# bioinfologics/w2rap-contigger

Hardware: AMD Instinct MI355X
Metric: step2_k60_canonical_kmers_per_s (higher is better)
Workload: dtype u64

## Files before the change

### w2rap_contigger_amd/csrc/step2_count.hip

```cpp
#include <algorithm>
#include <chrono>
#include <cstdlib>
#include <cstring>
#include <type_traits>
#include "ctx.h"

namespace w2 {

constexpr unsigned QSLOTS = 256;
template <bool MASK>
__global__ void __launch_bounds__(256) k_good_len(uint64_t n, const uint8_t* __restrict__ quals, const uint32_t* __restrict__ qmask,
                                                   const uint64_t* __restrict__ qoff, const uint32_t* __restrict__ len,
                                                   uint32_t min_qual, uint16_t* __restrict__ good,
                                                   unsigned long long* __restrict__ total_kmers,
                                                   uint32_t* __restrict__ max_len) {
    constexpr unsigned CH = 4096;
    __shared__ __attribute__((aligned(16))) uint16_t gbits[CH + 16];
    __shared__ unsigned long long s_sum[4];
    __shared__ uint32_t s_max[4];
    const uint64_t r0 = (uint64_t)blockIdx.x * blockDim.x;
    const uint64_t r = r0 + threadIdx.x;
    const uint64_t rend = r0 + blockDim.x < n ? r0 + blockDim.x : n;
    const uint64_t base0 = qoff[r0], endo = qoff[rend];
    const unsigned shift = MASK ? (unsigned)(base0 & 31) : (unsigned)((reinterpret_cast<uintptr_t>(quals) + base0) & 15);
// ... 949 lines not shown
                        const unsigned long long pos = gb + run + (unsigned)__builtin_popcountll(sm[j] & ((1ull << lane) - 1));
                        if (pos < solid_cap) { shi[pos] = keys[2 * i]; slo[pos] = keys[2 * i + 1]; scc[pos] = vals[j] & 0xFFFFu; }
                        keys[2 * i] = EMPTY; keys[2 * i + 1] = EMPTY;
                    }
                    run += (unsigned)__builtin_popcountll(sm[j]);
                }
            }
            tick(5);
            if (sp == 0) break;
            __syncthreads();
        }
    }
    __syncthreads();
    if (tid == 0) { misc[K3_BASELO] = (uint32_t)pend_base; misc[K3_BASEHI] = (uint32_t)(pend_base >> 32); }
    __syncthreads();
    {
        const uint32_t nprev = misc[K3_NPREV];
        const unsigned long long pk = (unsigned long long)misc[K3_BASELO] | ((unsigned long long)misc[K3_BASEHI] << 32);
        const unsigned long long gb = pk & SMASK;
        for (unsigned i = tid; i < nprev; i += THREADS)
            if (gb + i < solid_cap) { shi[gb + i] = sthi[i]; slo[gb + i] = stlo[i]; scc[gb + i] = stcc[i]; }
        if (tid == 0 && nprev && chunk_start && (pk >> 40) < chunk_cap) { chunk_start[pk >> 40] = gb; chunk_cnt[pk >> 40] = nprev; }
    }
    for (unsigned i = tid; i < 101; i += THREADS) if (lhist[i]) atomicAdd(&ghist[i], (unsigned long long)lhist[i]);
    for (int o = 32; o > 0; o >>= 1) my_distinct += __shfl_down(my_distinct, o);
    if (lane == 0 && my_distinct) atomicAdd(&counters[1], my_distinct);
    if (PROF && tid == 0) { for (int i = 0; i < 6; ++i) atomicAdd(&counters[106 + i], pt[i]); atomicAdd(&counters[112], ptmax);
                            for (int i = 0; i < 5; ++i) atomicAdd(&counters[113 + i], wt[i]); }
    if (PROF && lane == 0) atomicAdd(&counters[124 + wv], wcount);
}

#ifdef W2RAP_FP_TS9
constexpr unsigned FP_TS = REC_DWORDS | 1u;
#else
constexpr unsigned FP_TS = REC_DWORDS;
#endif
__device__ inline unsigned fp_tile_index(unsigned d) { return FP_TS == REC_DWORDS ? d : d + d / REC_DWORDS; }
template <unsigned THREADS, unsigned TILE_, unsigned SC_>
struct FpCfg {
    static constexpr unsigned CAP = 4096, LOG_CAP = 12, NW = THREADS / 64;
    static constexpr unsigned TILE = TILE_;
    static constexpr unsigned ROUNDS = (TILE + THREADS - 1) / THREADS;
    static constexpr unsigned MAXK = 16384, MAXWIN = MAXK / 64;
    static constexpr unsigned PFREC = TILE < 512 ? TILE : 512;
    static constexpr unsigned NPF = (PFREC * REC_DWORDS + THREADS - 1) / THREADS;
    static constexpr unsigned SC = SC_;
    static constexpr unsigned QCAP = 128;
    static constexpr unsigned MAXSEG = 16;
    static constexpr unsigned LIMIT = CAP - THREADS - 8 < 3072 ? CAP - THREADS - 8 : 3072;
    static constexpr unsigned PER = CAP / THREADS;
    static constexpr unsigned OCAP = CAP;
    static constexpr unsigned LDS = 3 * MAXSEG * 8 +
                                    (2 * CAP + TILE * FP_TS + 8 + MAXK / 32 + 2 + MAXWIN + 2 + 2 * SC + NW * QCAP + 3 * (MAXSEG + 1) + 32 + 4 + 104 + 16 + 40 + (OCAP + 1) / 2) * 4;
    static_assert(TILE < 1023 && ROUNDS * NW <= 16 && (1u << LOG_CAP) == CAP, "FpCfg");
};
enum { FP_FILL = 0, FP_OVF, FP_CNT, FP_BASELO, FP_BASEHI, FP_WIN, FP_DEPTH };
#ifndef W2RAP_FP_TICKETS
#define W2RAP_FP_TICKETS 4
#endif
constexpr uint32_t FP_TICKETS = W2RAP_FP_TICKETS;
static_assert((FP_TICKETS & (FP_TICKETS - 1)) == 0, "FP_TICKETS");

struct FpInst {
    uint32_t s[4];
    uint32_t e0, e3;
};
__device__ inline FpInst fp_fetch(const uint32_t* tile, unsigned rec, unsigned idx) {
    const uint32_t* wp = tile + rec * FP_TS;
    const unsigned q0 = (idx + REC_HB / 2) >> 4, sh = ((idx + REC_HB / 2) & 15u) * 2u;
    const uint32_t d0 = wp[q0], d1 = wp[1 + q0], d2 = wp[2 + q0], d3 = wp[3 + q0], d4 = wp[4 + q0];
    FpInst x;
    const uint32_t e0 = __funnelshift_r(d0, d1, sh), e1 = __funnelshift_r(d1, d2, sh), e2 = __funnelshift_r(d2, d3, sh), e3 = __funnelshift_r(d3, d4, sh);
    x.s[0] = __funnelshift_r(e0, e1, 2); x.s[1] = (e1 >> 2) & 0x0FFFFFFFu;
    x.s[2] = __funnelshift_r(e1, e2, 30); x.s[3] = __funnelshift_r(e2, e3, 30) & 0x0FFFFFFFu;
    x.e0 = e0; x.e3 = e3;
    return x;
}
struct FpKey { uint64_t hi, lo; bool rc; uint32_t f[4]; };
__device__ inline FpKey fp_key(const FpInst& x) {
    auto rev2_32 = [](uint32_t v) { v = __brev(v); return ((v & 0x55555555u) << 1) | ((v >> 1) & 0x55555555u); };
    const uint32_t a0 = rev2_32(x.s[0]), b0 = rev2_32(x.s[1]), a1 = rev2_32(x.s[2]), b1 = rev2_32(x.s[3]);
    FpKey k;
    k.f[0] = a0 >> 4; k.f[1] = __funnelshift_r(b0, a0, 4); k.f[2] = a1 >> 4; k.f[3] = __funnelshift_r(b1, a1, 4);
    const uint64_t khi_f = ((uint64_t)k.f[0] << 32) | k.f[1], klo_f = ((uint64_t)k.f[2] << 32) | k.f[3];
    const uint64_t khi_r = ((uint64_t)(~x.s[3] & 0x0FFFFFFFu) << 32) | (uint32_t)~x.s[2], klo_r = ((uint64_t)(~x.s[1] & 0x0FFFFFFFu) << 32) | (uint32_t)~x.s[0];
    k.rc = khi_r != khi_f ? khi_r < khi_f : klo_r < klo_f;
    k.hi = k.rc ? khi_r : khi_f; k.lo = k.rc ? klo_r : klo_f;
    return k;
}
__device__ inline uint32_t fp_hash(const FpKey& k) {
    const uint32_t fa = (uint32_t)k.hi ^ (uint32_t)(k.lo >> 32), fb = (uint32_t)(k.hi >> 32) ^ (uint32_t)k.lo;
    return (fa + ((fb << 16) | (fb >> 16))) * 0x9E3779B1u;
}
__device__ inline bool fp_same(const uint32_t* tile, unsigned ref, const FpInst& x, const FpKey& k) {
    const FpInst r = fp_fetch(tile, ref >> 6, ref & 63u);
    const uint32_t same = (r.s[0] ^ x.s[0]) | (r.s[1] ^ x.s[1]) | (r.s[2] ^ x.s[2]) | (r.s[3] ^ x.s[3]);
    const uint32_t opp = ((r.s[3] ^ k.f[0]) | 0xF0000000u) & (r.s[2] ^ k.f[1]) & ((r.s[1] ^ k.f[2]) | 0xF0000000u) & (r.s[0] ^ k.f[3]);
    return same == 0u || opp == 0xFFFFFFFFu;
}

template <unsigned THREADS, unsigned MINW, unsigned TILE_, unsigned SC_>
__global__ void __launch_bounds__(THREADS, MINW) k_count_fp(uint32_t nb, uint32_t b_lo, uint32_t b_hi, uint32_t nseg, const uint64_t* __restrict__ roff,
                                                            const uint32_t* __restrict__ recs, uint32_t min_freq, uint32_t* __restrict__ queue,
                                                            uint64_t* __restrict__ shi, uint64_t* __restrict__ slo, uint32_t* __restrict__ scc, uint64_t solid_cap,
                                                            unsigned long long* __restrict__ counters, unsigned long long* __restrict__ ghist,
                                                            uint64_t* __restrict__ chunk_start, uint32_t* __restrict__ chunk_cnt, uint32_t chunk_cap,
                                                            uint32_t* __restrict__ defer , uint32_t defer_cap,
                                                            uint32_t fill_limit , uint32_t solid_limit ,
                                                            uint8_t* __restrict__ sctx, uint8_t* __restrict__ unres, uint32_t* __restrict__ nbr ) {
    constexpr unsigned long long SMASK = (1ull << 40) - 1;
    using C = FpCfg<THREADS, TILE_, SC_>;
    constexpr unsigned CAP = C::CAP, NW = C::NW, TILE = C::TILE, ROUNDS = C::ROUNDS, NPF = C::NPF, SC = C::SC, MAXSEG = C::MAXSEG, PER = C::PER, QCAP = C::QCAP,
                       MAXK = C::MAXK, MAXWIN = C::MAXWIN;
    constexpr uint32_t EMPTY = 0xFFFFFFFFu;
    extern __shared__ __attribute__((aligned(16))) unsigned char smem[];
    uint64_t* segbase = reinterpret_cast<uint64_t*>(smem);
    uint32_t* tab = reinterpret_cast<uint32_t*>(segbase + 3 * MAXSEG);
    uint32_t* cc = tab + CAP;
    uint32_t* tile = cc + CAP;
    uint32_t* bv32 = tile + TILE * FP_TS + 8;
    uint32_t* Bw = bv32 + MAXK / 32 + 2;
    uint32_t* stcc = Bw + MAXWIN + 2;
    uint32_t* stref = stcc + SC;
    uint32_t* qref = stref + SC + (threadIdx.x >> 6) * QCAP;
    uint32_t* segdpre = stref + SC + NW * QCAP;
    uint32_t* wtot = segdpre + 3 * (MAXSEG + 1);
    uint32_t* bq = wtot + 32;
    uint32_t* lhist = bq + 4;
    uint32_t* misc = lhist + 104;
    uint32_t* stk = misc + 16;
    uint16_t* olist = reinterpret_cast<uint16_t*>(stk + 40);
    const unsigned tid = threadIdx.x, lane = tid & 63, wv = tid >> 6;

    auto seg_load = [&](uint32_t bb, uint64_t& r0, uint32_t& cnt) {
        r0 = 0; cnt = 0;
        if (tid < nseg && bb < b_hi) {
            const uint64_t a = roff[(uint64_t)tid * nb + bb], e = roff[(uint64_t)tid * nb + bb + 1];
            r0 = a; cnt = e - a < (1ull << 20) ? (uint32_t)(e - a) : (1u << 20);
        }
    };
    auto seg_store = [&](unsigned q, uint64_t r0, uint32_t cnt) {
        uint32_t incl = cnt;
#pragma unroll
        for (int o = 1; o < 64; o <<= 1) { uint32_t v = __shfl_up(incl, o); if ((int)lane >= o) incl += v; }
        const uint32_t tot = (uint32_t)__builtin_amdgcn_readlane((int)incl, 63);
        const uint32_t ex = incl - cnt;
        if (lane < nseg) { segdpre[q * (MAXSEG + 1) + lane] = ex * REC_DWORDS; segbase[q * MAXSEG + lane] = (r0 - ex) * REC_DWORDS; }
        if (lane == 0) segdpre[q * (MAXSEG + 1) + nseg] = tot * REC_DWORDS;
    };
    auto stream_dword = [&](unsigned q, const uint32_t* dp, const uint32_t (&bnd)[7], uint32_t d) -> uint32_t {
        unsigned s = 0;
        if (nseg <= 8) {
#pragma unroll
            for (unsigned i = 0; i < 7; ++i) s += d >= bnd[i] ? 1u : 0u;
        } else while (d >= dp[s + 1]) ++s;
        return recs[segbase[q * MAXSEG + s] + d];
    };
    auto tile_load = [&](unsigned q, uint32_t (&v)[NPF]) {
        const uint32_t* dp = segdpre + q * (MAXSEG + 1);
        const uint32_t dall = dp[nseg];
        const uint32_t dend = dall < C::PFREC * REC_DWORDS ? dall : C::PFREC * REC_DWORDS;
        uint32_t bnd[7];
#pragma unroll
        for (unsigned i = 0; i < 7; ++i) bnd[i] = (i + 1 < nseg && nseg <= 8) ? dp[i + 1] : 0xFFFFFFFFu;
#pragma unroll
        for (unsigned j = 0; j < NPF; ++j) {
            const uint32_t d = j * THREADS + tid;
            v[j] = d < dend ? stream_dword(q, dp, bnd, d) : 0u;
        }
    };
    auto tile_store = [&](const uint32_t (&v)[NPF]) {
#pragma unroll
        for (unsigned j = 0; j < NPF; ++j) { const unsigned i = j * THREADS + tid; if (i < C::PFREC * REC_DWORDS) tile[fp_tile_index(i)] = v[j]; }
    };
    auto tile_rest = [&](unsigned q) {
        if (TILE <= C::PFREC) return;
        const uint32_t* dp = segdpre + q * (MAXSEG + 1);
        const uint32_t dall = dp[nseg];
        const uint32_t dend = dall < TILE * REC_DWORDS ? dall : TILE * REC_DWORDS;
        uint32_t bnd[7];
#pragma unroll
        for (unsigned i = 0; i < 7; ++i) bnd[i] = (i + 1 < nseg && nseg <= 8) ? dp[i + 1] : 0xFFFFFFFFu;
        for (uint32_t d = C::PFREC * REC_DWORDS + tid; d < dend; d += THREADS) tile[fp_tile_index(d)] = stream_dword(q, dp, bnd, d);
    };
    auto ctx_of = [&](const FpInst& x, bool rc, uint32_t hdr, unsigned idx) -> unsigned {
        const unsigned rnk_ = (hdr & 63u) + 1u;
        const bool hasp = (idx > 0) | ((hdr & 64u) != 0), hass = (idx + 1 < rnk_) | ((hdr & 128u) != 0);
        const unsigned shl_p = (x.e0 & 3u) ^ (rc ? 3u : 4u), shl_s = ((x.e3 >> 26) & 3u) ^ (rc ? 7u : 0u);
        return (hasp ? 1u << shl_p : 0u) | (hass ? 1u << shl_s : 0u);
    };

    for (unsigned i = tid; i < CAP; i += THREADS) { tab[i] = EMPTY; cc[i] = 0; }
    for (unsigned i = tid; i < MAXK / 32 + 2; i += THREADS) bv32[i] = 0;
    for (unsigned i = tid; i < TILE * FP_TS + 8; i += THREADS) tile[i] = 0;
    for (unsigned i = tid; i < 104; i += THREADS) lhist[i] = 0;
    if (tid < 16) misc[tid] = 0;
    if (tid == 0) {
        const uint32_t t0 = atomicAdd(queue, 3u), nbk = b_hi - b_lo;
        bq[0] = t0 < nbk ? b_lo + t0 : NONE32; bq[1] = t0 + 1 < nbk ? b_lo + t0 + 1 : NONE32; bq[2] = t0 + 2 < nbk ? b_lo + t0 + 2 : NONE32; bq[3] = NONE32;
    }
    __syncthreads();
    if (wv == 0) {
        uint64_t r0; uint32_t cnt;
        seg_load(bq[0], r0, cnt); seg_store(0, r0, cnt);
        seg_load(bq[1], r0, cnt); seg_store(1, r0, cnt);
    }
    __syncthreads();
    uint32_t pf[NPF];
    tile_load(0, pf);
    unsigned long long my_distinct = 0;
    unsigned qn = 0;
    uint32_t tick4 = 0;

    auto drain = [&](unsigned cnt) -> unsigned {
        wave_lds_fence();
        const bool live = lane < cnt;
        const unsigned ref = live ? qref[qn - cnt + lane] : 0u;
        const unsigned rec = ref >> 6, idx = ref & 63u;
        const FpInst x = fp_fetch(tile, rec, idx);
        const FpKey k = fp_key(x);
        const unsigned ctx = ctx_of(x, k.rc, tile[rec * FP_TS], idx);
        const uint32_t h1 = fp_hash(k), tag = (h1 >> 5) & 0xFFFFu;
        unsigned s = (h1 >> (33 - C::LOG_CAP)) << 1;
        bool isnew = false;
        if (live) {
            bool ok = false;
            int budget = (int)CAP;
            for (;;) {
                uint32_t a = ld32(&tab[s]);
                if (a == EMPTY) {
                    a = atomicCAS(&tab[s], EMPTY, (tag << 16) | ref);
                    if (a == EMPTY) { isnew = true; ok = true; break; }
                }
                if ((a >> 16) == tag && fp_same(tile, a & 0xFFFFu, x, k)) { ok = true; break; }
                s = (s + 1) & (CAP - 1);
                if (--budget <= 0) break;
            }
            if (ok) { atomicAdd(&cc[s], 1u); atomicOr(&cc[s], ctx << 24); }
            else st32(&misc[FP_OVF], 1u);
        }
        qn -= cnt;
        wave_lds_fence();
        return (unsigned)__builtin_popcountll(__ballot(isnew));
    };

    for (uint32_t it = 0;; ++it) {
        const uint32_t b = (uint32_t)__builtin_amdgcn_readfirstlane((int)ld32(&bq[it & 3]));
        if (b >= b_hi) break;
        const unsigned q = it % 3;
        const uint32_t nrec = (uint32_t)__builtin_amdgcn_readfirstlane((int)segdpre[q * (MAXSEG + 1) + nseg]) / REC_DWORDS;
        bool skip = nrec > TILE;
        tile_store(pf);
        if (!skip) tile_rest(q);
        uint32_t la_b = 0;
        if (tid == 0) {
            if ((it & (FP_TICKETS - 1u)) == 0) tick4 = atomicAdd(queue, FP_TICKETS);
            const uint32_t t = tick4 + (it & (FP_TICKETS - 1u));
            la_b = t < b_hi - b_lo ? b_lo + t : NONE32;
        }
        uint64_t la_r0 = 0; uint32_t la_cnt = 0;
        if (wv == 0) seg_load(ld32(&bq[(it + 2) & 3]), la_r0, la_cnt);
        tile_load((it + 1) % 3, pf);
        __syncthreads();
        unsigned nkr[ROUNDS], inclr[ROUNDS];
#pragma unroll
        for (unsigned r = 0; r < ROUNDS; ++r) {
            const unsigned rec = r * THREADS + tid;
            nkr[r] = (!skip && rec < nrec) ? (tile[rec * FP_TS] & 63u) + 1u : 0u;
            inclr[r] = wave_scan64(nkr[r]);
            if (lane == 63) wtot[r * NW + wv] = inclr[r];
        }
        if (tid == 0) { misc[FP_WIN] = 2 * NW; stk[0] = 0; stk[1] = 1; misc[FP_DEPTH] = 1; }
        __syncthreads();
        const unsigned wsum = lane < ROUNDS * NW ? wtot[lane] : 0u, wsc = row_scan16(wsum);
        const int wvu = __builtin_amdgcn_readfirstlane((int)wv);
        const unsigned total = (unsigned)__builtin_amdgcn_readlane((int)wsc, ROUNDS * NW - 1);
        skip |= total > MAXK;
#pragma unroll
        for (unsigned r = 0; r < ROUNDS; ++r) {
            const unsigned base = (unsigned)__builtin_amdgcn_readlane((int)wsc, r * NW + wvu) - (unsigned)__builtin_amdgcn_readlane((int)wsum, r * NW + wvu);
            if (nkr[r] && !skip) {
                const unsigned e = base + inclr[r] - nkr[r], rec = r * THREADS + tid;
                atomicOr(&bv32[e >> 5], 1u << (e & 31));
                const unsigned w1 = (e + 63) >> 6;
                if (64 * w1 < e + nkr[r]) Bw[w1] = (rec << 16) | e;
            }
        }
        __syncthreads();
        const unsigned nwin = skip ? 0u : (total + 63) / 64;
        bool first_pass = true;
        for (;;) {
        const unsigned sp = (unsigned)__builtin_amdgcn_readfirstlane((int)ld32(&misc[FP_DEPTH])) - 1u;
        const uint32_t cls = (uint32_t)__builtin_amdgcn_readfirstlane((int)stk[2 * sp]), P = (uint32_t)__builtin_amdgcn_readfirstlane((int)stk[2 * sp + 1]);
        {
            uint32_t fill_seen = (uint32_t)__builtin_amdgcn_readfirstlane((int)ld32(&misc[FP_FILL])),
                     ovf_seen = (uint32_t)__builtin_amdgcn_readfirstlane((int)ld32(&misc[FP_OVF]));
            const unsigned wv_s = (unsigned)wvu;
            uint32_t nM0 = 0, nM1 = 0, nB = 0;
            { const unsigned w0 = wv_s < nwin ? wv_s : 0u; nM0 = bv32[2 * w0]; nM1 = bv32[2 * w0 + 1]; nB = Bw[w0]; }
            const uint64_t lane_le = ~0ull >> (63 - lane);
            const uint32_t lane_lt_lo = lane < 32 ? (1u << lane) - 1u : 0xFFFFFFFFu, lane_lt_hi = lane < 32 ? 0u : (1u << (lane - 32)) - 1u;
            unsigned wnext = wv_s + NW;
            for (unsigned w = wv_s; w < nwin;) {
                if (ovf_seen) break;
                if (fill_seen >= fill_limit) { if (lane == 0) st32(&misc[FP_OVF], 1u); break; }
                const uint32_t fill_ld = ld32(&misc[FP_FILL]), ovf_ld = ld32(&misc[FP_OVF]);
                uint32_t wdraw = 0;
                if (lane == 0) wdraw = atomicAdd(&misc[FP_WIN], 1u);
                const uint32_t M0 = nM0, M1 = nM1, Bv = nB;
                { const unsigned wn = wnext < nwin ? wnext : w; nM0 = bv32[2 * wn]; nM1 = bv32[2 * wn + 1]; nB = Bw[wn]; }
                const unsigned g = w * 64 + lane;
                const bool active = g < total;
                const uint32_t mle0 = M0 & (uint32_t)lane_le, mle1 = M1 & (uint32_t)(lane_le >> 32);
                const unsigned c = (unsigned)__builtin_popcount(mle0 & ~1u) + (unsigned)__builtin_popcount(mle1);
                const unsigned top = mle1 ? 63u - (unsigned)__builtin_clz(mle1) : 31u - (unsigned)__builtin_clz(mle0 | 1u);
                const unsigned idx = active ? lane - (c ? top : (Bv & 0xFFFFu) - w * 64) : 0u;
                const unsigned rec = active ? (Bv >> 16) + c : 0u;
                const uint32_t hdr = tile[rec * FP_TS];
                const FpInst x = fp_fetch(tile, rec, idx);
                const FpKey k = fp_key(x);
                const unsigned ctx = ctx_of(x, k.rc, hdr, idx);
                const uint32_t h1 = fp_hash(k), tag = (h1 >> 5) & 0xFFFFu;
                const unsigned s0 = (h1 >> (33 - C::LOG_CAP)) << 1;
                const unsigned myref = (rec << 6) | idx;
                const uint64_t ab = ld64(reinterpret_cast<const uint64_t*>(tab + s0));
                const uint32_t a0 = (uint32_t)ab, a1 = (uint32_t)(ab >> 32);
                const bool m0 = ((a0 >> 16) == tag) & (a0 != EMPTY), m1 = ((a1 >> 16) == tag) & (a1 != EMPTY);
                const bool second = !m0 & (m1 | ((a0 != EMPTY) & (a1 == EMPTY)));
                const uint32_t a = second ? a1 : a0;
                const unsigned s = s0 + (second ? 1u : 0u);
                const bool mine = active & (((h1 >> 2) & (P - 1)) == cls);
                const bool tagm = mine & (m0 | m1);
                const bool hit = tagm & fp_same(tile, tagm ? (a & 0xFFFFu) : myref, x, k);
                const bool want = mine & !tagm & (a == EMPTY);
                const uint32_t old = atomicCAS(&tab[s], EMPTY, want ? ((tag << 16) | myref) : EMPTY);
                const bool won = want & (old == EMPTY);
                const bool done = hit | won;
                atomicAdd(&cc[s], done ? 1u : 0u);
                atomicOr(&cc[s], done ? ctx << 24 : 0u);
                const bool parked = mine & !done;
                unsigned nnew = (unsigned)__builtin_popcountll(__ballot(won));
                {
                    const unsigned long long pm = __ballot(parked);
                    const unsigned below = (unsigned)__builtin_popcount((uint32_t)pm & lane_lt_lo) + (unsigned)__builtin_popcount((uint32_t)(pm >> 32) & lane_lt_hi);
                    const unsigned npark = (unsigned)__builtin_popcountll(pm);
                    qref[qn + (parked ? below : npark + lane - below)] = myref;
                    qn += npark;
                    if (qn >= 64) nnew += drain(64);
                }
                if (nnew && lane == 0) atomicAdd(&misc[FP_FILL], nnew);
                fill_seen = (uint32_t)__builtin_amdgcn_readfirstlane((int)fill_ld); ovf_seen = (uint32_t)__builtin_amdgcn_readfirstlane((int)ovf_ld);
                w = wnext; wnext = (uint32_t)__builtin_amdgcn_readfirstlane((int)wdraw);
            }
            unsigned nnew = 0;
            while (qn) nnew += drain(qn < 64 ? qn : 64);
            if (nnew && lane == 0) atomicAdd(&misc[FP_FILL], nnew);
        }
        if (first_pass) {
            if (wv == 0) seg_store((it + 2) % 3, la_r0, la_cnt);
            if (tid == 0) st32(&bq[(it + 3) & 3], la_b);
            first_pass = false;
        }
        if (tid == 0) {
            misc[FP_CNT] = 0;
            if (skip) misc[FP_OVF] = 1;
        }
        __syncthreads();
        bool deferred = ld32(&misc[FP_OVF]) != 0;
        static_assert(PER % 4 == 0, "PER");
        uint32_t occm = 0, nsol = 0;
        if (!deferred) {
            const u32x4* c4 = reinterpret_cast<const u32x4*>(cc + tid * PER);
#pragma unroll
            for (unsigned j4 = 0; j4 < PER / 4; ++j4) {
                const u32x4 v4 = c4[j4];
#pragma unroll
                for (unsigned j = 0; j < 4; ++j) {
                    const uint32_t cnt = v4[j] & 0xFFFFFFu;
                    occm |= (cnt != 0 ? 1u : 0u) << (4 * j4 + j);
                    nsol += (cnt != 0 && cnt >= min_freq) ? 1u : 0u;
                }
            }
        }
        const unsigned nocc = (unsigned)__builtin_popcount(occm);
        const unsigned i_occ = wave_scan64(nocc), i_sol = wave_scan64(nsol);
        if (lane == 63) { wtot[wv] = i_occ; wtot[16 + wv] = i_sol; }
        __syncthreads();
        const unsigned ws_o = lane < NW ? wtot[lane] : 0u, wc_o = row_scan16(ws_o), ws_s = lane < NW ? wtot[16 + lane] : 0u, wc_s = row_scan16(ws_s);
        const unsigned tot_occ = (unsigned)__builtin_amdgcn_readlane((int)wc_o, NW - 1), tot = (unsigned)__builtin_amdgcn_readlane((int)wc_s, NW - 1);
        deferred |= tot > solid_limit;
        if (deferred) {
            for (unsigned i = tid; i < CAP; i += THREADS) { tab[i] = EMPTY; cc[i] = 0; }
            if (tid == 0) {
                if (skip) {
                    const uint32_t at = atomicAdd(&defer[0], 1u);
                    if (at < defer_cap) defer[2 + at] = b; else counters[3] = 3;
                    misc[FP_DEPTH] = sp;
                } else if (P >= (1u << 16)) { counters[3] = 1; misc[FP_DEPTH] = sp; }
                else { atomicAdd(&counters[2], 1ull); stk[2 * sp] = cls + P; stk[2 * sp + 1] = 2 * P; stk[2 * sp + 2] = cls; stk[2 * sp + 3] = 2 * P; misc[FP_DEPTH] = sp + 2; }
// ... 51 lines not shown
                if (have && gb + i < solid_cap) { shi[gb + i] = k.hi; slo[gb + i] = k.lo; scc[gb + i] = ccv; }
                if (sctx) {
                    constexpr uint32_t NONE = 0xFFFFFFFFu, PAL = 0xFFFFFFFEu;
                    unsigned c = (ccv >> 8) & 0xFFu, un = 0;
                    uint32_t ns = NONE, np_ = NONE;
                    const Kmer kk{k.hi, k.lo};
                    for (unsigned rest = have ? c : 0u; __any(rest != 0);) {
                        if (rest) {
                            const unsigned t = (unsigned)__builtin_ctz(rest);
                            rest &= rest - 1;
                            Kmer nk = t < 4 ? kmer_succ(kk, t & 3) : kmer_pred(kk, t & 3);
                            const bool r = kmer_canon(nk);
                            FpInst nx; FpKey nkk;
                            const uint64_t lh = rev2_64(nk.hi) >> 4, ll = rev2_64(nk.lo) >> 4;
                            nx.s[0] = (uint32_t)lh; nx.s[1] = (uint32_t)(lh >> 32); nx.s[2] = (uint32_t)ll; nx.s[3] = (uint32_t)(ll >> 32); nx.e0 = 0; nx.e3 = 0;
                            nkk.hi = nk.hi; nkk.lo = nk.lo; nkk.rc = false;
                            nkk.f[0] = (uint32_t)(nk.hi >> 32); nkk.f[1] = (uint32_t)nk.hi; nkk.f[2] = (uint32_t)(nk.lo >> 32); nkk.f[3] = (uint32_t)nk.lo;
                            const uint32_t h1 = fp_hash(nkk), tag = (h1 >> 5) & 0xFFFFu;
                            unsigned s = (h1 >> (33 - C::LOG_CAP)) << 1;
                            int found = -1;
                            for (int budget = (int)CAP; budget > 0; --budget) {
                                const uint32_t a = tab[s];
                                if (a == EMPTY) break;
                                if ((a >> 16) == tag && fp_same(tile, a & 0xFFFFu, nx, nkk)) { found = (int)s; break; }
                                s = (s + 1) & (CAP - 1);
                            }
                            if (found < 0) un |= 1u << t;
                            else {
                                const uint32_t v = cc[found];
                                if (v & 0x80000000u) {
                                    const uint32_t id = kmer_is_pal(nk) ? PAL : (uint32_t)(2 * (gb + (v & 0xFFFFu)) + (r ? 1u : 0u));
                                    if (t < 4) ns = id; else np_ = id;
                                } else c &= ~(1u << t);
                            }
                        }
                    }
                    if (have && gb + i < solid_cap) {
                        const unsigned long long gi = gb + i;
                        sctx[gi] = (uint8_t)c; unres[gi] = (uint8_t)un;
                        nbr[2 * gi] = (!(un & 15u) && popc4(c & 15) != 1) ? NONE : ns;
                        nbr[2 * gi + 1] = (!(un >> 4) && popc4(c >> 4) != 1) ? NONE : np_;
                    }
                }
            }
        }
        __syncthreads();
        if (sctx) {
            for (unsigned i = tid; i < tot_occ; i += THREADS) { const unsigned slot = olist[i]; cc[slot] = 0; tab[slot] = EMPTY; }
            if (sp != 0) __syncthreads();
        }
        if (sp == 0) break;
        }
        for (unsigned i = tid; i < 2 * nwin + 2; i += THREADS) bv32[i] = 0;
    }
    __syncthreads();
    for (unsigned i = tid; i < 101; i += THREADS) if (lhist[i]) atomicAdd(&ghist[i], (unsigned long long)lhist[i]);
    for (int o = 32; o > 0; o >>= 1) my_distinct += __shfl_down(my_distinct, o);
    if (lane == 0 && my_distinct) atomicAdd(&counters[1], my_distinct);
}

__global__ void __launch_bounds__(256) k_table_insert(uint64_t i0, uint64_t S, const uint64_t* __restrict__ shi, const uint64_t* __restrict__ slo,
                                                       Slot* __restrict__ table, uint64_t mask) {
    uint64_t i = i0 + (uint64_t)blockIdx.x * blockDim.x + threadIdx.x;
    if (i >= S) return;
    const uint64_t h = kmer_hash(Kmer{shi[i], slo[i]});
    const Slot v = slot_make(h, i);
    uint64_t s = h & mask;
    while (atomicCAS(&table[s], SLOT_EMPTY, v) != SLOT_EMPTY) s = (s + 1) & mask;
}

template <unsigned U> struct PlCfg { static constexpr unsigned CAP = 256 * U, SLOTS = 512 * U, BITS = U == 2 ? 10 : U == 4 ? 11 : 12; };
template <unsigned BITS>
__device__ inline unsigned pl_hash(Kmer k) {
    const uint32_t fa = (uint32_t)k.hi ^ (uint32_t)(k.lo >> 32), fb = (uint32_t)(k.hi >> 32) ^ (uint32_t)k.lo;
    return ((fa + ((fb << 16) | (fb >> 16))) * 0x9E3779B1u) >> (32 - BITS);
}
template <class Id, unsigned U = 2>
__global__ void __launch_bounds__(256) k_prune_local(uint64_t nchunks, const uint64_t* __restrict__ cstart, const uint32_t* __restrict__ ccnt,
                                                      const uint64_t* __restrict__ shi, const uint64_t* __restrict__ slo,
                                                      const uint32_t* __restrict__ scc, uint8_t* __restrict__ sctx,
                                                      Id* __restrict__ nbr, uint8_t* __restrict__ unres) {
    constexpr Id NONE = NodeId<Id>::NONE, PAL = NodeId<Id>::PAL;
    constexpr unsigned PL_CAP = PlCfg<U>::CAP, PL_SLOTS = PlCfg<U>::SLOTS, PL_BITS = PlCfg<U>::BITS;
    __shared__ uint64_t khi[PL_SLOTS], klo[PL_SLOTS];
    __shared__ uint16_t kix[PL_SLOTS];
    const unsigned tid = threadIdx.x;
    auto load_desc = [&](uint64_t ch, uint64_t& st_, uint32_t& cn_) {
        st_ = 0; cn_ = 0;
        if (ch < nchunks) { st_ = cstart[ch]; cn_ = ccnt[ch]; if (cn_ > PL_CAP) cn_ = 0; }
    };
    auto load_keys = [&](uint64_t st_, uint32_t cn_, Kmer (&k_)[U], unsigned (&c_)[U]) {
#pragma unroll
        for (unsigned u = 0; u < U; ++u) {
            const unsigned j = tid + 256 * u;
            k_[u] = Kmer{0, 0}; c_[u] = 0;
            if (j < cn_) { k_[u] = Kmer{shi[st_ + j], slo[st_ + j]}; c_[u] = (scc[st_ + j] >> 8) & 0xFF; }
        }
    };
    uint64_t st_c, st_n; uint32_t cn_c, cn_n;
    Kmer nx[U]; unsigned ncx[U];
    load_desc(blockIdx.x, st_c, cn_c);
    load_keys(st_c, cn_c, nx, ncx);
    load_desc((uint64_t)blockIdx.x + gridDim.x, st_n, cn_n);
    for (uint64_t ch = blockIdx.x; ch < nchunks; ch += gridDim.x) {
        const uint64_t start = st_c;
        const uint32_t cnt = cn_c;
        Kmer mine[U]; unsigned cm[U];
#pragma unroll
        for (unsigned u = 0; u < U; ++u) { mine[u] = nx[u]; cm[u] = ncx[u]; }
        st_c = st_n; cn_c = cn_n;
        load_keys(st_c, cn_c, nx, ncx);
        load_desc(ch + 2 * (uint64_t)gridDim.x, st_n, cn_n);
// ... 462 lines not shown
    const unsigned NS = c.cs_planned;
    const uint32_t nbl = c.cs_nbl, nseg = c.cs_nseg;
    unsigned long long* d_cnt = c.cs_cnt;
#ifndef W2RAP_QUEUE_AT
#define W2RAP_QUEUE_AT 144
#endif
    uint32_t* d_queue = reinterpret_cast<uint32_t*>(d_cnt + W2RAP_QUEUE_AT);
    uint32_t b_lo, b_hi;
    count_slice_bounds(c, k, &b_lo, &b_hi);
    auto slice_done = [&]() -> int {
        W2_HIP(hipMemcpyAsync(c.h_pinned + k, d_cnt + 4, 8, hipMemcpyDeviceToHost, st));
        W2_HIP(hipEventCreateWithFlags(&c.cs_ev[k], hipEventDisableTiming));
        W2_HIP(hipEventRecord(c.cs_ev[k], st));
        c.cs_ns = k + 1;
        return 0;
    };
    auto launch = [&](auto kern, unsigned lds, unsigned threads, unsigned blocks_per_cu) -> int {
        W2_HIP(hipFuncSetAttribute(reinterpret_cast<const void*>(kern), hipFuncAttributeMaxDynamicSharedMemorySize, lds));
        unsigned grid = (unsigned)std::min<uint64_t>(b_hi - b_lo, (uint64_t)c.sm_count * blocks_per_cu);
        if (k || c.pass) W2_HIP(hipMemsetAsync(d_queue, 0, 4, st));
        LAUNCH(c, "k_count_buckets", kern, dim3(grid ? grid : 1), dim3(threads), lds, nbl, b_lo, b_hi, nseg, c.cs_off, c.cs_recs, c.min_freq, d_queue,
               c.d_shi, c.d_slo, c.d_scc, c.solid_cap, d_cnt + 4, d_cnt + 8, c.d_chunk_start, c.d_chunk_cnt, c.cs_chunk_cap, (const uint32_t*)nullptr, 0u);
        W2_HIP(hipGetLastError());
        return slice_done();
    };
    auto launch_fp = [&](auto kern, unsigned lds, unsigned threads, unsigned blocks_per_cu, uint32_t fp_limit, uint32_t fp_sc) -> int {
        W2_HIP(hipFuncSetAttribute(reinterpret_cast<const void*>(kern), hipFuncAttributeMaxDynamicSharedMemorySize, lds));
        auto list_kern = k_count_buckets<COUNT_CAP, COUNT_THREADS>;
        W2_HIP(hipFuncSetAttribute(reinterpret_cast<const void*>(list_kern), hipFuncAttributeMaxDynamicSharedMemorySize, (int)K3Cfg<COUNT_CAP, COUNT_THREADS>::LDS));
        const unsigned grid = (unsigned)std::min<uint64_t>(b_hi - b_lo, (uint64_t)c.sm_count * blocks_per_cu);
        if (k || c.pass) W2_HIP(hipMemsetAsync(d_queue, 0, 4, st));
        if (k == 0) W2_HIP(hipMemsetAsync(c.cs_defer, 0, 8, st));
        uint32_t fill_limit = fp_limit, solid_limit = fp_sc;
        if (const char* t = getenv("W2RAP_TEST_FP_LIMIT")) { if (test_hook("W2RAP_TEST_FP_LIMIT")) fill_limit = std::min<uint32_t>(fill_limit, (uint32_t)std::max(1, atoi(t))); }
        if (const char* t = getenv("W2RAP_TEST_FP_SC")) { if (test_hook("W2RAP_TEST_FP_SC")) solid_limit = std::min<uint32_t>(solid_limit, (uint32_t)std::max(1, atoi(t))); }
        LAUNCH(c, "k_count_fp", kern, dim3(grid ? grid : 1), dim3(threads), lds, nbl, b_lo, b_hi, nseg, c.cs_off, c.cs_recs, c.min_freq, d_queue,
               c.d_shi, c.d_slo, c.d_scc, c.solid_cap, d_cnt + 4, d_cnt + 8, c.d_chunk_start, c.d_chunk_cnt, c.cs_chunk_cap, c.cs_defer, nbl, fill_limit, solid_limit,
               c.fused_prune ? c.d_sctx : (uint8_t*)nullptr, c.fused_prune ? c.d_unres : (uint8_t*)nullptr, c.fused_prune ? (uint32_t*)c.d_nbr : (uint32_t*)nullptr);
        W2_HIP(hipGetLastError());
        if (k + 1 == NS && c.fused_prune) W2_HIP(hipMemcpyAsync(c.h_pinned + 20, d_cnt + 4, 8, hipMemcpyDeviceToHost, st));
        if (k + 1 == NS) {
            const unsigned lgrid = (unsigned)std::min<uint64_t>(nbl, (uint64_t)c.sm_count);
            constexpr unsigned list_lds = K3Cfg<COUNT_CAP, COUNT_THREADS>::LDS;
            LAUNCH(c, "k_count_buckets", list_kern, dim3(lgrid ? lgrid : 1), dim3(COUNT_THREADS), list_lds, nbl, 0u, nbl, nseg, c.cs_off,
                   c.cs_recs, c.min_freq, c.cs_defer + 1, c.d_shi, c.d_slo, c.d_scc, c.solid_cap, d_cnt + 4, d_cnt + 8, c.d_chunk_start, c.d_chunk_cnt, c.cs_chunk_cap,
                   (const uint32_t*)c.cs_defer, nbl);
            W2_HIP(hipGetLastError());
        }
        return slice_done();
    };
    const char* v = getenv("W2RAP_K3");
    int cfg = v ? atoi(v) : 22;
    if (cfg >= 20 && nseg > FpCfg<512, 512, 1024>::MAXSEG) cfg = 0;
    if (cfg == 20) W2_TRY(launch_fp(k_count_fp<512, 4, 640, 768>, FpCfg<512, 640, 768>::LDS, 512, 2, FpCfg<512, 640, 768>::LIMIT, 768));
    else if (cfg == 21) W2_TRY(launch_fp(k_count_fp<1024, 8, 576, 512>, FpCfg<1024, 576, 512>::LDS, 1024, 2, FpCfg<1024, 576, 512>::LIMIT, 512));
    else if (cfg == 22) W2_TRY(launch_fp(k_count_fp<512, 4, 512, 1024>, FpCfg<512, 512, 1024>::LDS, 512, 2, FpCfg<512, 512, 1024>::LIMIT, 1024));
    else if (cfg == 23) W2_TRY(launch_fp(k_count_fp<1024, 4, 576, 1024>, FpCfg<1024, 576, 1024>::LDS, 1024, 1, FpCfg<1024, 576, 1024>::LIMIT, 1024));
    else if (cfg == 24) W2_TRY(launch_fp(k_count_fp<512, 4, 576, 1024>, FpCfg<512, 576, 1024>::LDS, 512, 2, FpCfg<512, 576, 1024>::LIMIT, 1024));
    else if (cfg == 1) W2_TRY(launch(k_count_buckets<2048, 512>, K3Cfg<2048, 512>::LDS, 512, 2));
    else if (cfg == 2) W2_TRY(launch(k_count_buckets<4096, 512>, K3Cfg<4096, 512>::LDS, 512, 1));
    else if (cfg == 3) W2_TRY(launch(k_count_buckets<1024, 256>, K3Cfg<1024, 256>::LDS, 256, 4));
    else if (cfg == 5) W2_TRY(launch(k_count_buckets<2048, 1024, false, false, 8>, K3Cfg<2048, 1024, false>::LDS, 1024, 2));
    else if (cfg == 8) W2_TRY(launch(k_count_buckets<4096, 1024, false, false, 1>, K3Cfg<4096, 1024, false>::LDS, 1024, 1));
    else if (cfg == 9) W2_TRY(launch(k_count_buckets<COUNT_CAP, COUNT_THREADS, true>, K3Cfg<COUNT_CAP, COUNT_THREADS>::LDS, COUNT_THREADS, 1));
    else W2_TRY(launch(k_count_buckets<COUNT_CAP, COUNT_THREADS>, K3Cfg<COUNT_CAP, COUNT_THREADS>::LDS, COUNT_THREADS, 1));
    return 0;
}

int count_buckets_slice(Ctx& c, unsigned k, uint64_t* n_solid, uint64_t* n_chunks) {
    if (k >= c.cs_ns) { c.err = "count_records_slice: slice not launched"; return W2RAP_E_ARG; }
    W2_HIP(hipEventSynchronize(c.cs_ev[k]));
    const uint64_t w = c.h_pinned[k];
    if (n_solid) *n_solid = std::min<uint64_t>(w & ((1ull << 40) - 1), c.solid_cap);
    if (n_chunks) *n_chunks = std::min<uint64_t>(w >> 40, c.cs_chunk_cap);
    return 0;
}

int count_buckets_finish(Ctx& c) {
    hipStream_t st = c.stream;
    if (!c.cs_planned || c.cs_ns != c.cs_planned) { c.err = "count_records_end: not every slice has been launched"; return W2RAP_E_STATE; }
    unsigned long long h_all[160];
    W2_HIP(hipMemcpyAsync(h_all, c.cs_cnt, sizeof(h_all), hipMemcpyDeviceToHost, st));
    W2_HIP(hipStreamSynchronize(st));
    for (unsigned k = 0; k < c.cs_ns; ++k) (void)hipEventDestroy(c.cs_ev[k]);
    c.cs_ns = 0; c.cs_planned = 0;
    if (c.pass + 1 < c.npass) c.pass_cnt = c.cs_cnt;
    else { c.release(c.cs_cnt); c.pass_cnt = nullptr; c.pass = 0; c.npass = 1; }
    c.release(c.cs_off); c.cs_cnt = nullptr; c.cs_off = nullptr;
    if (getenv("W2RAP_TRACE") && c.cs_defer) {
        uint32_t nd = 0;
        (void)hipMemcpy(&nd, c.cs_defer, 4, hipMemcpyDeviceToHost);
        fprintf(stderr, "[w2rap] k_count_fp deferred %u buckets (all slices) to k_count_buckets\n", nd);
    }
    if (c.cs_defer) { c.release(c.cs_defer); c.cs_defer = nullptr; }
    if (getenv("W2RAP_TRACE") && h_all[111])
        fprintf(stderr, "[w2rap] k_count_buckets wave-0 clocks per block: stage-in %.0f, count %.0f, barrier A %.0f, flush+scan %.0f, barrier B %.0f, staging %.0f; slowest wave's count %.0f (x%u blocks, %u buckets)\n",
                (double)h_all[110] / c.sm_count, (double)h_all[111] / c.sm_count, (double)h_all[112] / c.sm_count, (double)h_all[113] / c.sm_count,
                (double)h_all[114] / c.sm_count, (double)h_all[115] / c.sm_count, (double)h_all[116] / c.sm_count, (unsigned)c.sm_count, 0u);
    if (getenv("W2RAP_TRACE") && h_all[128]) {
        fprintf(stderr, "[w2rap] k_count_buckets count-phase clocks per block, by wave:");
        for (int w = 0; w < 16; ++w) fprintf(stderr, " %.1fM", (double)h_all[128 + w] / c.sm_count / 1e6);
        fprintf(stderr, "\n");
    }
    if (getenv("W2RAP_TRACE") && h_all[121])
        fprintf(stderr, "[w2rap] k_count_buckets wave-0 clocks per window: loads %.0f, extract+hash %.0f, probe %.0f, atomics %.0f (%.0f windows per block)\n",
                (double)h_all[117] / h_all[121], (double)h_all[118] / h_all[121], (double)h_all[119] / h_all[121], (double)h_all[120] / h_all[121],
                (double)h_all[121] / c.sm_count);
    if (h_all[7]) { c.err = "k_count_buckets: a bucket did not fit the LDS table after 2^16-way splitting"; return W2RAP_E_LIMIT; }
    c.S = h_all[4] & ((1ull << 40) - 1); c.D = h_all[5];
    c.nchunks = c.cs_chunk_cap ? std::min<uint64_t>(h_all[4] >> 40, c.cs_chunk_cap) : 0;
    for (int i = 0; i < 101; ++i) c.hist[i] = h_all[8 + i];
// ... 296 lines not shown
```

Baseline: 41.32 billion.

## Deduplicate identical read records per tile before k-mer counting with multiplicity weights

Adds a per-tile LDS hash table that detects byte-identical read records, drops the duplicates from k-mer enumeration, and carries their multiplicity into the count atomics and queued references. The aim is to avoid re-hashing and re-inserting the same k-mers for duplicate reads, which are common in sequencing data. The cost is an extra hashing and probing pass per record, more LDS, a fixed VGPR cap of 60 on the new kernel, and packing multiplicity into the upper 16 bits of prefix-scan and queue values. It is on by default and can be turned off with W2RAP_FP_DEDUP=0.

```diff
diff --git a/w2rap_contigger_amd/csrc/step2_count.hip b/w2rap_contigger_amd/csrc/step2_count.hip
--- a/w2rap_contigger_amd/csrc/step2_count.hip
+++ b/w2rap_contigger_amd/csrc/step2_count.hip
@@ -1025,7 +1025,11 @@
     static constexpr unsigned OCAP = CAP;
     static constexpr unsigned LDS = 3 * MAXSEG * 8 +
                                     (2 * CAP + TILE * FP_TS + 8 + MAXK / 32 + 2 + MAXWIN + 2 + 2 * SC + NW * QCAP + 3 * (MAXSEG + 1) + 32 + 4 + 104 + 16 + 40 + (OCAP + 1) / 2) * 4;
+    static constexpr unsigned DT = TILE <= 512 ? 1024 : 2048, LOG_DT = TILE <= 512 ? 10 : 11;
+    static constexpr unsigned DAREA = DT + (TILE + 1) / 2;
+    static constexpr unsigned LDS_DEDUP = LDS + TILE * 4;
     static_assert(TILE < 1023 && ROUNDS * NW <= 16 && (1u << LOG_CAP) == CAP, "FpCfg");
+    static_assert(DT >= 2 * TILE && DAREA <= 2 * SC + NW * QCAP && TILE * 64 < 65536 && (OCAP & 1) == 0, "FpCfg: record dedup");
 };
 enum { FP_FILL = 0, FP_OVF, FP_CNT, FP_BASELO, FP_BASEHI, FP_WIN, FP_DEPTH };
 #ifndef W2RAP_FP_TICKETS
@@ -1072,15 +1076,43 @@
     return same == 0u || opp == 0xFFFFFFFFu;
 }
 
-template <unsigned THREADS, unsigned MINW, unsigned TILE_, unsigned SC_>
-__global__ void __launch_bounds__(THREADS, MINW) k_count_fp(uint32_t nb, uint32_t b_lo, uint32_t b_hi, uint32_t nseg, const uint64_t* __restrict__ roff,
-                                                            const uint32_t* __restrict__ recs, uint32_t min_freq, uint32_t* __restrict__ queue,
-                                                            uint64_t* __restrict__ shi, uint64_t* __restrict__ slo, uint32_t* __restrict__ scc, uint64_t solid_cap,
-                                                            unsigned long long* __restrict__ counters, unsigned long long* __restrict__ ghist,
-                                                            uint64_t* __restrict__ chunk_start, uint32_t* __restrict__ chunk_cnt, uint32_t chunk_cap,
-                                                            uint32_t* __restrict__ defer , uint32_t defer_cap,
-                                                            uint32_t fill_limit , uint32_t solid_limit ,
-                                                            uint8_t* __restrict__ sctx, uint8_t* __restrict__ unres, uint32_t* __restrict__ nbr ) {
+template <unsigned DT, unsigned LOG_DT>
+__device__ inline bool fp_dedup(const uint32_t* tile, uint32_t* dtab, uint32_t* dmul, unsigned rec) {
+    const uint32_t* wp = tile + rec * FP_TS;
+    uint32_t w[REC_DWORDS];
+#pragma unroll
+    for (unsigned i = 0; i < REC_DWORDS; ++i) w[i] = wp[i];
+    auto rotl = [](uint32_t v, unsigned n) { return __funnelshift_l(v, v, n); };
+    uint32_t x = w[0], y = w[REC_DWORDS - 1];
+#pragma unroll
+    for (unsigned i = 1; i + 1 < REC_DWORDS; i += 2) { x = rotl(x, 9) + w[i]; y = rotl(y, 13) ^ w[i + 1]; }
+    uint32_t h = (x + rotl(y, 16)) * 0x9E3779B1u;
+    h ^= h >> 15;
+    unsigned s = (h * 0x85EBCA6Bu) >> (32 - LOG_DT);
+    for (;;) {
+        uint32_t a = ld32(&dtab[s]);
+        if (a == 0u) { a = atomicCAS(&dtab[s], 0u, rec + 1u); if (a == 0u) return false; }
+        const uint32_t* hp = tile + (a - 1u) * FP_TS;
+        uint32_t d = 0;
+#pragma unroll
+        for (unsigned i = 0; i < REC_DWORDS; ++i) d |= hp[i] ^ w[i];
+        if (d == 0u) { atomicAdd(&dmul[(a - 1u) >> 1], 1u << (16u * ((a - 1u) & 1u))); return true; }
+        s = (s + 1u) & (DT - 1u);
+    }
+}
+
+#define W2_FP_PARAMS                                                                                                                                  \
+    uint32_t nb, uint32_t b_lo, uint32_t b_hi, uint32_t nseg, const uint64_t* __restrict__ roff, const uint32_t* __restrict__ recs, uint32_t min_freq, \
+    uint32_t* __restrict__ queue, uint64_t* __restrict__ shi, uint64_t* __restrict__ slo, uint32_t* __restrict__ scc, uint64_t solid_cap,              \
+    unsigned long long* __restrict__ counters, unsigned long long* __restrict__ ghist, uint64_t* __restrict__ chunk_start,                            \
+    uint32_t* __restrict__ chunk_cnt, uint32_t chunk_cap, uint32_t* __restrict__ defer , uint32_t defer_cap, \
+    uint32_t fill_limit , uint32_t solid_limit ,                                               \
+    uint8_t* __restrict__ sctx, uint8_t* __restrict__ unres, uint32_t* __restrict__ nbr
+#define W2_FP_ARGS                                                                                                                                    \
+    nb, b_lo, b_hi, nseg, roff, recs, min_freq, queue, shi, slo, scc, solid_cap, counters, ghist, chunk_start, chunk_cnt, chunk_cap, defer, defer_cap, \
+    fill_limit, solid_limit, sctx, unres, nbr
+template <unsigned THREADS, unsigned TILE_, unsigned SC_, bool DEDUP>
+__device__ __forceinline__ void count_fp_body(W2_FP_PARAMS) {
     constexpr unsigned long long SMASK = (1ull << 40) - 1;
     using C = FpCfg<THREADS, TILE_, SC_>;
     constexpr unsigned CAP = C::CAP, NW = C::NW, TILE = C::TILE, ROUNDS = C::ROUNDS, NPF = C::NPF, SC = C::SC, MAXSEG = C::MAXSEG, PER = C::PER, QCAP = C::QCAP,
@@ -1103,6 +1135,9 @@
     uint32_t* misc = lhist + 104;
     uint32_t* stk = misc + 16;
     uint16_t* olist = reinterpret_cast<uint16_t*>(stk + 40);
+    uint32_t* rinfo = reinterpret_cast<uint32_t*>(olist + C::OCAP);
+    uint32_t* dtab = stcc;
+    uint32_t* dmul = stcc + C::DT;
     const unsigned tid = threadIdx.x, lane = tid & 63, wv = tid >> 6;
 
     auto seg_load = [&](uint32_t bb, uint64_t& r0, uint32_t& cnt) {
@@ -1168,6 +1203,7 @@
     for (unsigned i = tid; i < TILE * FP_TS + 8; i += THREADS) tile[i] = 0;
     for (unsigned i = tid; i < 104; i += THREADS) lhist[i] = 0;
     if (tid < 16) misc[tid] = 0;
+    if (DEDUP) for (unsigned i = tid; i < C::DAREA; i += THREADS) dtab[i] = 0;
     if (tid == 0) {
         const uint32_t t0 = atomicAdd(queue, 3u), nbk = b_hi - b_lo;
         bq[0] = t0 < nbk ? b_lo + t0 : NONE32; bq[1] = t0 + 1 < nbk ? b_lo + t0 + 1 : NONE32; bq[2] = t0 + 2 < nbk ? b_lo + t0 + 2 : NONE32; bq[3] = NONE32;
@@ -1188,8 +1224,8 @@
     auto drain = [&](unsigned cnt) -> unsigned {
         wave_lds_fence();
         const bool live = lane < cnt;
-        const unsigned ref = live ? qref[qn - cnt + lane] : 0u;
-        const unsigned rec = ref >> 6, idx = ref & 63u;
+        const uint32_t qv = live ? qref[qn - cnt + lane] : 0u;
+        const unsigned ref = qv & 0xFFFFu, rec = ref >> 6, idx = ref & 63u;
         const FpInst x = fp_fetch(tile, rec, idx);
         const FpKey k = fp_key(x);
         const unsigned ctx = ctx_of(x, k.rc, tile[rec * FP_TS], idx);
@@ -1209,7 +1245,7 @@
                 s = (s + 1) & (CAP - 1);
                 if (--budget <= 0) break;
             }
-            if (ok) { atomicAdd(&cc[s], 1u); atomicOr(&cc[s], ctx << 24); }
+            if (ok) { atomicAdd(&cc[s], DEDUP ? qv >> 16 : 1u); atomicOr(&cc[s], ctx << 24); }
             else st32(&misc[FP_OVF], 1u);
         }
         qn -= cnt;
@@ -1239,24 +1275,29 @@
 #pragma unroll
         for (unsigned r = 0; r < ROUNDS; ++r) {
             const unsigned rec = r * THREADS + tid;
-            nkr[r] = (!skip && rec < nrec) ? (tile[rec * FP_TS] & 63u) + 1u : 0u;
-            inclr[r] = wave_scan64(nkr[r]);
+            bool dup = false;
+            if (DEDUP && !skip && r * THREADS + (tid & ~63u) < nrec)
+                if (rec < nrec) dup = fp_dedup<C::DT, C::LOG_DT>(tile, dtab, dmul, rec);
+            nkr[r] = (!skip && rec < nrec && !dup) ? (tile[rec * FP_TS] & 63u) + 1u : 0u;
+            inclr[r] = wave_scan64(DEDUP ? nkr[r] | (nkr[r] ? 1u << 16 : 0u) : nkr[r]);
             if (lane == 63) wtot[r * NW + wv] = inclr[r];
         }
         if (tid == 0) { misc[FP_WIN] = 2 * NW; stk[0] = 0; stk[1] = 1; misc[FP_DEPTH] = 1; }
         __syncthreads();
         const unsigned wsum = lane < ROUNDS * NW ? wtot[lane] : 0u, wsc = row_scan16(wsum);
         const int wvu = __builtin_amdgcn_readfirstlane((int)wv);
-        const unsigned total = (unsigned)__builtin_amdgcn_readlane((int)wsc, ROUNDS * NW - 1);
+        const unsigned total = (unsigned)__builtin_amdgcn_readlane((int)wsc, ROUNDS * NW - 1) & (DEDUP ? 0xFFFFu : ~0u);
         skip |= total > MAXK;
 #pragma unroll
         for (unsigned r = 0; r < ROUNDS; ++r) {
             const unsigned base = (unsigned)__builtin_amdgcn_readlane((int)wsc, r * NW + wvu) - (unsigned)__builtin_amdgcn_readlane((int)wsum, r * NW + wvu);
             if (nkr[r] && !skip) {
-                const unsigned e = base + inclr[r] - nkr[r], rec = r * THREADS + tid;
+                const unsigned pe = base + inclr[r], rec = r * THREADS + tid;
+                const unsigned e = (DEDUP ? pe & 0xFFFFu : pe) - nkr[r], j = DEDUP ? (pe >> 16) - 1u : rec;
                 atomicOr(&bv32[e >> 5], 1u << (e & 31));
                 const unsigned w1 = (e + 63) >> 6;
-                if (64 * w1 < e + nkr[r]) Bw[w1] = (rec << 16) | e;
+                if (64 * w1 < e + nkr[r]) Bw[w1] = (j << 16) | e;
+                if (DEDUP) rinfo[j] = rec | ((1u + ((dmul[rec >> 1] >> (16u * (rec & 1u))) & 0xFFFFu)) << 16);
             }
         }
         __syncthreads();
@@ -1288,7 +1329,9 @@
                 const unsigned c = (unsigned)__builtin_popcount(mle0 & ~1u) + (unsigned)__builtin_popcount(mle1);
                 const unsigned top = mle1 ? 63u - (unsigned)__builtin_clz(mle1) : 31u - (unsigned)__builtin_clz(mle0 | 1u);
                 const unsigned idx = active ? lane - (c ? top : (Bv & 0xFFFFu) - w * 64) : 0u;
-                const unsigned rec = active ? (Bv >> 16) + c : 0u;
+                const unsigned rj = active ? (Bv >> 16) + c : 0u;
+                const uint32_t inf = DEDUP ? rinfo[rj] : rj;
+                const unsigned rec = inf & 0xFFFFu;
                 const uint32_t hdr = tile[rec * FP_TS];
                 const FpInst x = fp_fetch(tile, rec, idx);
                 const FpKey k = fp_key(x);
@@ -1309,7 +1352,7 @@
                 const uint32_t old = atomicCAS(&tab[s], EMPTY, want ? ((tag << 16) | myref) : EMPTY);
                 const bool won = want & (old == EMPTY);
                 const bool done = hit | won;
-                atomicAdd(&cc[s], done ? 1u : 0u);
+                atomicAdd(&cc[s], done ? (DEDUP ? inf >> 16 : 1u) : 0u);
                 atomicOr(&cc[s], done ? ctx << 24 : 0u);
                 const bool parked = mine & !done;
                 unsigned nnew = (unsigned)__builtin_popcountll(__ballot(won));
@@ -1317,7 +1360,7 @@
                     const unsigned long long pm = __ballot(parked);
                     const unsigned below = (unsigned)__builtin_popcount((uint32_t)pm & lane_lt_lo) + (unsigned)__builtin_popcount((uint32_t)(pm >> 32) & lane_lt_hi);
                     const unsigned npark = (unsigned)__builtin_popcountll(pm);
-                    qref[qn + (parked ? below : npark + lane - below)] = myref;
+                    qref[qn + (parked ? below : npark + lane - below)] = DEDUP ? myref | (inf & 0xFFFF0000u) : myref;
                     qn += npark;
                     if (qn >= 64) nnew += drain(64);
                 }
@@ -1475,12 +1518,19 @@
         if (sp == 0) break;
         }
         for (unsigned i = tid; i < 2 * nwin + 2; i += THREADS) bv32[i] = 0;
+        if (DEDUP) for (unsigned i = tid; i < C::DAREA; i += THREADS) dtab[i] = 0;
     }
     __syncthreads();
     for (unsigned i = tid; i < 101; i += THREADS) if (lhist[i]) atomicAdd(&ghist[i], (unsigned long long)lhist[i]);
     for (int o = 32; o > 0; o >>= 1) my_distinct += __shfl_down(my_distinct, o);
     if (lane == 0 && my_distinct) atomicAdd(&counters[1], my_distinct);
 }
+template <unsigned THREADS, unsigned MINW, unsigned TILE_, unsigned SC_>
+__global__ void __launch_bounds__(THREADS, MINW) k_count_fp(W2_FP_PARAMS) { count_fp_body<THREADS, TILE_, SC_, false>(W2_FP_ARGS); }
+template <unsigned THREADS, unsigned MINW, unsigned TILE_, unsigned SC_>
+__global__ void __attribute__((amdgpu_num_vgpr(60))) __launch_bounds__(THREADS, MINW) k_count_fp_dedup(W2_FP_PARAMS) { count_fp_body<THREADS, TILE_, SC_, true>(W2_FP_ARGS); }
+#undef W2_FP_PARAMS
+#undef W2_FP_ARGS
 
 __global__ void __launch_bounds__(256) k_table_insert(uint64_t i0, uint64_t S, const uint64_t* __restrict__ shi, const uint64_t* __restrict__ slo,
                                                        Slot* __restrict__ table, uint64_t mask) {
@@ -2049,11 +2099,17 @@
     const char* v = getenv("W2RAP_K3");
     int cfg = v ? atoi(v) : 22;
     if (cfg >= 20 && nseg > FpCfg<512, 512, 1024>::MAXSEG) cfg = 0;
-    if (cfg == 20) W2_TRY(launch_fp(k_count_fp<512, 4, 640, 768>, FpCfg<512, 640, 768>::LDS, 512, 2, FpCfg<512, 640, 768>::LIMIT, 768));
-    else if (cfg == 21) W2_TRY(launch_fp(k_count_fp<1024, 8, 576, 512>, FpCfg<1024, 576, 512>::LDS, 1024, 2, FpCfg<1024, 576, 512>::LIMIT, 512));
-    else if (cfg == 22) W2_TRY(launch_fp(k_count_fp<512, 4, 512, 1024>, FpCfg<512, 512, 1024>::LDS, 512, 2, FpCfg<512, 512, 1024>::LIMIT, 1024));
-    else if (cfg == 23) W2_TRY(launch_fp(k_count_fp<1024, 4, 576, 1024>, FpCfg<1024, 576, 1024>::LDS, 1024, 1, FpCfg<1024, 576, 1024>::LIMIT, 1024));
-    else if (cfg == 24) W2_TRY(launch_fp(k_count_fp<512, 4, 576, 1024>, FpCfg<512, 576, 1024>::LDS, 512, 2, FpCfg<512, 576, 1024>::LIMIT, 1024));
+    const char* ddv = getenv("W2RAP_FP_DEDUP");
+    const bool dedup = !(ddv && atoi(ddv) == 0);
+#define W2_FP_SHAPE(T, W, TL, S, BPC)                                                                                                                  \
+    W2_TRY(dedup ? launch_fp(k_count_fp_dedup<T, W, TL, S>, FpCfg<T, TL, S>::LDS_DEDUP, T, BPC, FpCfg<T, TL, S>::LIMIT, S)                             \
+                 : launch_fp(k_count_fp<T, W, TL, S>, FpCfg<T, TL, S>::LDS, T, BPC, FpCfg<T, TL, S>::LIMIT, S))
+    if (cfg == 20) W2_FP_SHAPE(512, 4, 640, 768, 2);
+    else if (cfg == 21) W2_FP_SHAPE(1024, 8, 576, 512, 2);
+    else if (cfg == 22) W2_FP_SHAPE(512, 4, 512, 1024, 2);
+    else if (cfg == 23) W2_FP_SHAPE(1024, 4, 576, 1024, 1);
+    else if (cfg == 24) W2_FP_SHAPE(512, 4, 576, 1024, 2);
+#undef W2_FP_SHAPE
     else if (cfg == 1) W2_TRY(launch(k_count_buckets<2048, 512>, K3Cfg<2048, 512>::LDS, 512, 2));
     else if (cfg == 2) W2_TRY(launch(k_count_buckets<4096, 512>, K3Cfg<4096, 512>::LDS, 512, 1));
     else if (cfg == 3) W2_TRY(launch(k_count_buckets<1024, 256>, K3Cfg<1024, 256>::LDS, 256, 4));
```

Result: faster. 42.16 billion, median of 6 (+2.0%).
